# dsmyl6/OpenPyStruct

Hardware: AMD Instinct MI355X
Metric: beam FE solves/s (100-elem, batched) (higher is better)
Workload: dtype f64

## Files before the change

### openpystruct_amd/csrc/beam_fat.hip

```cpp
#include <hip/hip_runtime.h>
#include <stdint.h>

#include <type_traits>

#include "../../include/openpystruct_amd.h"
#include "beam_io.hpp"

namespace opsamd {

template <int PM>
struct FatAcc {
  const double* tab;
  const double* sI;
  const double* sF;
  FixPair bits;
  __device__ __forceinline__ ElemIn elem(int i) const {
    return ElemIn{tab[i], tab[PM + i], tab[2 * PM + i], tab[3 * PM + i], tab[4 * PM + i], tab[5 * PM + i], sI[i], sF[i]};
  }
  __device__ __forceinline__ FixPair fixbits() const { return bits; }
  __device__ __forceinline__ void fence() const { __asm__ volatile("" ::: "memory"); }
};

template <int M, bool FAT>
struct RowOut {
  double* sV; double* sM; double* sv;
  double th[M];
  double vr[FAT ? 1 : M];
  __device__ __forceinline__ void elem(int i, double Vv, double Mv) { sV[i] = Vv; sM[i] = Mv; }
  __device__ __forceinline__ void node(int i, double vv, double tt) {
    if constexpr (FAT) sv[i] = vv; else vr[i] = vv;
    th[i] = tt;
  }
};
template <int M, bool FAT>
struct ParkH {
  double* hx; double* hy;
  Vec2 r[FAT ? 1 : M];
  __device__ __forceinline__ void put(int i, const Vec2& h) {
    if constexpr (FAT) { hx[i] = h.x; hy[i] = h.y; } else r[i] = h;
  }
  __device__ __forceinline__ Vec2 get(int i) const {
    if constexpr (FAT) return Vec2{hx[i], hy[i]}; else return r[i];
  }
};

#ifdef OPS_AMD_TRACE
#define FAT_STAMP(k) (__builtin_amdgcn_sched_barrier(0), stamps[k] = __builtin_amdgcn_s_memrealtime(), __builtin_amdgcn_sched_barrier(0))
#else
#define FAT_STAMP(k) ((void)0)
#endif

struct FatIface {
  const IfacePiece* grp;
  __device__ __forceinline__ IfacePiece piece(int k) const { return grp[k]; }
  __device__ __forceinline__ Mat2 cup(int k) const { return grp[k].cup; }
  __device__ __forceinline__ void fence() const { __asm__ volatile("" ::: "memory"); }
};

template <int P, int M, bool RZ, bool FAT, int PF>
__device__ __forceinline__ void row_solve_lanes(const FatAcc<P * M>& acc, int g, int j, int& bad, RowOut<M, FAT>& out, ParkH<M, FAT>& hs,
                                                IfacePiece* pieces, unsigned lane, unsigned long long* stamps) {
  SegState<M> st;
  std::conditional_t<P == 16 && M == 7, KeepD<M>, KeepNone> keep;
  __asm__ volatile("" ::: "memory");
  seg_condense_pf<M, RZ>(st, acc, bad, keep);
  __asm__ volatile("" ::: "memory");
  FAT_STAMP(6);
  Vec2 uL, uR{0.0, 0.0};
  if constexpr (FAT) {
    pieces[lane] = make_piece<M, RZ>(st, acc.bits);
    __asm__ volatile("" ::: "memory");
    Vec2 u[P];
    iface_thomas<P>(FatIface{pieces + g * P}, u, bad);
    uL = u[0];
#pragma unroll
    for (int k = 1; k < P; ++k) {
      if (j == k) uL = u[k];
      if (j + 1 == k) uR = u[k];
    }
  } else {
    using X = Xch<P>;
    IfaceRow row;
    {
      const Mat2 cup = masked_cup<M, RZ>(st, acc.bits);
      const Sym2 pc = X::template from_minus<1>(st.Scc, (int)lane, j);
      const Vec2 pg = X::template from_minus<1>(st.gc, (int)lane, j);
      const Mat2 pb = X::template from_minus<1>(cup, (int)lane, j);
      row = make_row<M, RZ>(st, cup, pc, pg, pb, acc.bits);
    }
    cr_forward<P, 1>(row, (int)lane, j, bad);
    const Sym2 G = inv_spd(row.D, bad);
    uL = mul(G, row.f);
    if (j != 0) uL = Vec2{0.0, 0.0};
    cr_backward<P, cr_top_level(P)>(row, G, uL, (int)lane, j);
    uR = X::template from_plus<1>(uL, (int)lane, j);
  }
  __asm__ volatile("" ::: "memory");
  FAT_STAMP(7);
  seg_solve_pf<M, RZ, PF>(st, acc, uL, uR, out, hs, keep);
}

struct WordPick {
  bool q1, q2, q3;
  unsigned r;
  __device__ __forceinline__ explicit WordPick(int e0) : q1((e0 >> 5) == 1), q2((e0 >> 5) == 2), q3((e0 >> 5) == 3), r((unsigned)e0 & 31u) {}
};
__device__ __forceinline__ unsigned mask_window(unsigned long long lo, unsigned long long hi, const WordPick& w) {
  const unsigned w0 = (unsigned)lo, w1 = (unsigned)(lo >> 32), w2 = (unsigned)hi, w3 = (unsigned)(hi >> 32);
  unsigned a = w0, b = w1;
  a = w.q1 ? w1 : a;  b = w.q1 ? w2 : b;
  a = w.q2 ? w2 : a;  b = w.q2 ? w3 : b;
  a = w.q3 ? w3 : a;  b = w.q3 ? 0u : b;
  return __builtin_amdgcn_alignbit(b, a, w.r);
}

template <int P, int M, int WPS, bool FAT, bool SIZING>
__device__ __forceinline__ void beam_rows_body(const RowsHead& p, const RowsTail& t, const SizingArgs* sz) {
  constexpr int BPW = 64 / P;
  constexpr int LIVE = BPW * P;
  constexpr int PM = P * M;
  constexpr int NT = (PM + 63) / 64;
  constexpr int ROWS = BPW * PM;
  static_assert(PM <= 128 && PM % 2 == 0 && M + 1 <= 32, "row tiling limits");
  static_assert(FAT || (16 % P == 0 && LIVE == 64), "the lean mapping exchanges over DPP rows");
  constexpr int PF = FAT ? 3 : 1;
#ifdef OPS_AMD_ST
  constexpr int ST = OPS_AMD_ST;
#else
  constexpr int ST = 16;
#endif
  __shared__ double s_tab[6 * PM];
  __shared__ __attribute__((aligned(16))) double s_a[ROWS];
  __shared__ __attribute__((aligned(16))) double s_b[ROWS];
  __shared__ __attribute__((aligned(16))) double s_m[FAT ? ROWS : 2];
  __shared__ __attribute__((aligned(16))) double s_v[FAT ? ROWS : 2];
  __shared__ double s_dummy[M];
  static_assert((6 * PM + (FAT ? 4 : 2) * ROWS + M + 4) * 8 <= 160 * 1024 / (4 * WPS), "LDS per one-wave workgroup");
  static_assert(!FAT || (WPS == 1 && (6 * PM + 4 * ROWS) * 8 > 32 * 1024), "the fat tiling relies on LDS to keep a fifth wave off the CU");

  const unsigned lane = threadIdx.x;
  unsigned long long stamps[8] = {0, 0, 0, 0, 0, 0, 0, 0};
  FAT_STAMP(0);
  const int Ne = p.Ne, N = p.Ne + 1;
  const long I_bs = p.I_bs, Fy_bs = p.Fy_bs;
  const long beam0 = (long)blockIdx.x * BPW;
  const int nb = (p.B - beam0 < BPW) ? (int)(p.B - beam0) : BPW;
  if (SIZING && t.active) {
    unsigned any = 0;
    for (int b = 0; b < nb; ++b) any |= t.active[beam0 + b];
    if (!any) return;
  }
  const double tE = p.E[0], tw = p.wy[0];
  __builtin_amdgcn_sched_barrier(0);
  double tx0[NT], tx1[NT];
  {
    const __amdgpu_buffer_rsrc_t rx = make_rsrc(p.x, (unsigned)N * 8u);
#pragma unroll
    for (int k = 0; k < NT; ++k) {
      const unsigned e = lane + 64u * k;
      tx0[k] = buf_load_d(rx, e * 8u);
      tx1[k] = buf_load_d(rx, e * 8u + 8u);
    }
  }
  const int g_raw = lane / P, j = lane - g_raw * P, e0 = j * M;
  const bool live = (int)lane < LIVE;
  const int g = live ? g_raw : BPW - 1;
  const int hE = Ne >> 1, hN = N >> 1;
  double2 rI[BPW], rF[BPW];
  double tI = 0.0, tF = 0.0;
  {
    const __amdgpu_buffer_rsrc_t rsF = make_rsrc(p.Fy + beam0 * Fy_bs, (unsigned)(((long)(nb - 1) * Fy_bs + N) * 8));
    const unsigned oobF = (int)lane < hN ? lane * 16u : 0x40000000u;
    const unsigned tb = lane < (unsigned)nb ? lane : 0u;
    if constexpr (SIZING) {
      const __amdgpu_buffer_rsrc_t rsI = make_rsrc(static_cast<const float*>(p.I) + beam0 * Ne, (unsigned)(nb * Ne) * 4u);
      const unsigned oobI = (int)lane < hE ? lane * 8u : 0x40000000u;
#pragma unroll
      for (int b = 0; b < BPW; ++b) {
        const float2 f = __builtin_bit_cast(float2, __builtin_amdgcn_raw_buffer_load_b64(rsI, (int)((unsigned)(b * Ne) * 4u + oobI), 0, 0));
        rI[b] = make_double2((double)f.x, (double)f.y);
        rF[b] = buf_load_d2(rsF, (unsigned)(b * Fy_bs * 8) + oobF);
      }
      if (Ne & 1) tI = (double)__builtin_bit_cast(float, __builtin_amdgcn_raw_buffer_load_b32(rsI, (int)((tb * Ne + Ne - 1) * 4u), 0, 0));
    } else {
      const __amdgpu_buffer_rsrc_t rsI = make_rsrc(static_cast<const double*>(p.I) + beam0 * I_bs, (unsigned)(((long)(nb - 1) * I_bs + Ne) * 8));
      const unsigned oobI = (int)lane < hE ? lane * 16u : 0x40000000u;
#pragma unroll
      for (int b = 0; b < BPW; ++b) {
        rI[b] = buf_load_d2(rsI, (unsigned)(b * I_bs * 8) + oobI);
        rF[b] = buf_load_d2(rsF, (unsigned)(b * Fy_bs * 8) + oobF);
      }
      if (Ne & 1) tI = buf_load_d(rsI, (unsigned)((tb * I_bs + Ne - 1) * 8));
    }
    if (N & 1) tF = buf_load_d(rsF, (unsigned)((tb * Fy_bs + N - 1) * 8));
  }
  FAT_STAMP(5);
  unsigned char fb0, fb1;
  {
    const __amdgpu_buffer_rsrc_t rf = make_rsrc(t.fix, (unsigned)N);
    fb0 = __builtin_amdgcn_raw_buffer_load_b8(rf, (int)lane, 0, 0);
    fb1 = __builtin_amdgcn_raw_buffer_load_b8(rf, (int)(lane + 64u), 0, 0);
  }
#pragma unroll
  for (int k = 0; k < NT; ++k) {
    const unsigned e = lane + 64u * k;
    if (64 * (k + 1) <= Ne) {
      const double L = tx1[k] - tx0[k];
      const double rl = fast_rcp(L);
      const double c2 = 2.0 * tE * rl, pw = 0.5 * tw * L;
      const double c6 = 3.0 * c2 * rl, c12 = 2.0 * c6 * rl;
      const double mw = pw * L * (1.0 / 6.0);
      s_tab[0 * PM + e] = c2;  s_tab[1 * PM + e] = c6;  s_tab[2 * PM + e] = c12;
      s_tab[3 * PM + e] = rl;  s_tab[4 * PM + e] = pw;  s_tab[5 * PM + e] = mw;
    } else if (e < (unsigned)PM) {
      const bool real = (int)e < Ne, pad = (int)e > Ne;
      const double L = tx1[k] - tx0[k];
      const double rl0 = fast_rcp(real ? L : 1.0);
      const double c2r = 2.0 * tE * rl0, pwr = 0.5 * tw * L;
      const double rl = real ? rl0 : (pad ? 1.0 : 0.0);
      const double c2 = real ? c2r : (pad ? 2.0 : 0.0);
      const double c6 = 3.0 * c2 * rl, c12 = 2.0 * c6 * rl;
      const double pw = real ? pwr : 0.0, mw = pw * L * (1.0 / 6.0);
      s_tab[0 * PM + e] = c2;  s_tab[1 * PM + e] = c6;  s_tab[2 * PM + e] = c12;
      s_tab[3 * PM + e] = rl;  s_tab[4 * PM + e] = pw;  s_tab[5 * PM + e] = mw;
    }
  }
  FixPair bits;
  bool any_rz;
  {
    const unsigned long long v0 = __ballot(fb0 & 1), v1 = __ballot(fb1 & 1);
    const unsigned long long r0 = __ballot(fb0 & 2), r1 = __ballot(fb1 & 2);
    any_rz = (r0 | r1) != 0ull;
    const WordPick pick(e0);
    bits.v = mask_window(v0, v1, pick) & ((2u << M) - 1u);
    bits.t = any_rz ? mask_window(r0, r1, pick) & ((2u << M) - 1u) : 0u;
  }

  if (lane < M) s_dummy[lane] = 0.0;
#pragma unroll
  for (int k = 0; k < (ROWS / 2 + 63) / 64; ++k) {
    const unsigned idx = lane + 64u * k;
    if (k + 1 < (ROWS / 2 + 63) / 64 || idx < ROWS / 2) *reinterpret_cast<double2*>(&s_a[2 * idx]) = make_double2(1.0, 1.0);
  }
#pragma unroll
  for (int b = 0; b < BPW; ++b) {
    if ((int)lane < (b < nb ? hE : 0)) *reinterpret_cast<double2*>(&s_a[b * PM + 2 * lane]) = rI[b];
    if (lane < PM / 2) *reinterpret_cast<double2*>(&s_b[b * PM + 2 * lane]) = rF[b];
  }
  if ((Ne & 1) && (int)lane < nb) s_a[lane * PM + Ne - 1] = tI;
  if ((N & 1) && (int)lane < nb) s_b[lane * PM + N - 1] = tF;
  __syncthreads();
  FAT_STAMP(1);

  FatAcc<PM> acc;
  acc.tab = &s_tab[e0];
  acc.sI = &s_a[g * PM + e0];
  acc.sF = &s_b[g * PM + e0];
  acc.bits = bits;
  int bad = 0;
  RowOut<M, FAT> out;
  out.sV = live ? &s_b[g * PM + e0] : s_dummy;
  out.sM = live ? (FAT ? &s_m[g * PM + e0] : &s_a[g * PM + e0]) : s_dummy;
  out.sv = (FAT && live) ? &s_v[g * PM + e0] : s_dummy;
  ParkH<M, FAT> hs;
  hs.hx = out.sM; hs.hy = out.sv;
  static_assert(!FAT || 64 * sizeof(IfacePiece) <= ROWS * 8, "the interface pieces borrow the moment rows");
  IfacePiece* const pieces = reinterpret_cast<IfacePiece*>(s_m);
  if (any_rz) row_solve_lanes<P, M, true, FAT, PF>(acc, g, j, bad, out, hs, pieces, lane, stamps);
  else        row_solve_lanes<P, M, false, FAT, PF>(acc, g, j, bad, out, hs, pieces, lane, stamps);
  FAT_STAMP(2);

  const unsigned long long bal = __ballot(bad != 0 && live);
  const unsigned long long grp = (P == 64 ? ~0ull : ((1ull << (P % 64)) - 1ull)) << (g * P);
  const bool gbad = (bal & grp) != 0ull;
  if (bal != 0ull && gbad && live) {
    const double qnan = __builtin_nan("");
#pragma unroll
    for (int i = 0; i < M; ++i) {
      out.sV[i] = qnan; out.sM[i] = qnan; out.th[i] = qnan;
      if constexpr (FAT) out.sv[i] = qnan; else out.vr[i] = qnan;
    }
  }
  if (j == 0 && live && g < nb && t.status)
    __hip_atomic_store(&t.status[beam0 + g], gbad ? 1 : 0, __ATOMIC_RELAXED, __HIP_MEMORY_SCOPE_AGENT);
  double* const sth = live ? &s_a[g * PM + e0] : s_dummy;
  if constexpr (FAT) {
#pragma unroll
    for (int i = 0; i < M; ++i) sth[i] = out.th[i];
  }
  wave_lds_fence();
  if constexpr (SIZING) {
    static_assert(!SIZING || !FAT, "the fused epoch uses the lean mapping");
    CaseRegs<2> cr[BPW];
    bool on[BPW];
#pragma unroll
    for (int gb = 0; gb < BPW; ++gb) {
      on[gb] = gb < nb && sz->active[beam0 + gb] != 0;
      if (on[gb]) load_case<2>((int)lane, beam0 + gb, Ne, *sz, cr[gb]);
    }
#pragma unroll
    for (int gb = 0; gb < BPW; ++gb) {
      if (!on[gb]) continue;
      const double* Vb = &s_b[gb * PM];
      const double* Mb = &s_a[gb * PM];
      step_case<2>((int)lane, beam0 + gb, Ne, *sz, cr[gb], [&](int e) { return (float)Vb[e]; }, [&](int e) { return (float)Mb[e]; });
    }
    return;
  }

  const bool two = t.v != nullptr;
  auto read_rows = [&](double2 (&r)[BPW], double& tail, const double* s, int n_) {
    const unsigned lrow = (int)lane < (n_ >> 1) ? lane : 0u;
#pragma unroll
    for (int b = 0; b < BPW; ++b) r[b] = *reinterpret_cast<const double2*>(&s[b * PM + 2 * lrow]);
    tail = s[((int)lane < nb ? lane : 0u) * PM + n_ - 1];
  };
  auto store_rows = [&](auto aux, double* dst, const double2 (&r)[BPW], double tail, int n_) {
    constexpr int AUX = decltype(aux)::value;
    const __amdgpu_buffer_rsrc_t rs = make_rsrc(dst + beam0 * n_, (unsigned)(nb * n_) * 8u);
    const unsigned off = (int)lane < (n_ >> 1) ? lane * 16u : 0x40000000u;
#pragma unroll
    for (int b = 0; b < BPW; ++b)
      buf_store_d2<AUX>(rs, (unsigned)(b * n_) * 8u + off, r[b]);
    if ((n_ & 1) && (int)lane < nb) buf_store_d<AUX>(rs, (unsigned)(lane * n_ + n_ - 1) * 8u, tail);
  };
  auto all_rows = [&](auto aux) {
    double2 ra[BPW], rb[BPW];
    double ta, tb;
    read_rows(ra, ta, s_b, Ne);
    read_rows(rb, tb, FAT ? s_m : s_a, Ne);
    if constexpr (FAT) {
      store_rows(aux, t.V, ra, ta, Ne);
      if (two) read_rows(ra, ta, s_v, N);
      store_rows(aux, t.M, rb, tb, Ne);
      if (two) {
        read_rows(rb, tb, s_a, N);
        store_rows(aux, t.v, ra, ta, N);
        store_rows(aux, t.theta, rb, tb, N);
      }
    } else {
      if (two) {
        wave_lds_fence();
        double* const svv = live ? &s_b[g * PM + e0] : s_dummy;
#pragma unroll
        for (int i = 0; i < M; ++i) { svv[i] = out.vr[i]; sth[i] = out.th[i]; }
      }
      store_rows(aux, t.V, ra, ta, Ne);
      store_rows(aux, t.M, rb, tb, Ne);
      if (two) {
        wave_lds_fence();
        read_rows(ra, ta, s_b, N);
        read_rows(rb, tb, s_a, N);
        store_rows(aux, t.v, ra, ta, N);
        store_rows(aux, t.theta, rb, tb, N);
      }
    }
  };
  if (t.stream_out) all_rows(std::integral_constant<int, 2>{});
  else              all_rows(std::integral_constant<int, ST>{});
#ifdef OPS_AMD_TRACE
  if (t.trace && lane == 0) {
    FAT_STAMP(3);
    stamps[4] = __builtin_amdgcn_s_getreg((4 << 0) | (0 << 6) | ((16 - 1) << 11));
    unsigned long long* q = t.trace + 8 * (unsigned long long)blockIdx.x;
#pragma unroll
    for (int k = 0; k < 8; ++k) q[k] = stamps[k];
  }
#endif
}

template <int P, int M, int WPS, bool FAT>
__global__ __launch_bounds__(64, WPS) void beam_rows_kernel(int Ne, int B, const void* I, const double* Fy, unsigned I_bs, unsigned Fy_bs,
                                                           const double* x, const double* E, const double* wy, const RowsTail t) {
  beam_rows_body<P, M, WPS, FAT, false>(RowsHead{Ne, B, I, Fy, I_bs, Fy_bs, x, E, wy}, t, nullptr);
}
template <int P, int M, int WPS>
__global__ __launch_bounds__(64, WPS) void beam_rows_sizing_kernel(const RowsHead h, const RowsTail t, const SizingArgs sz) {
  beam_rows_body<P, M, WPS, false, true>(h, t, &sz);
}

const FatTiling kFatTilings[] = {
    {6, 17, "beam_rows_kernel<6, 17, 1, true>"},
    {16, 7, "beam_rows_kernel<16, 7, 3, false>"},
    {8, 13, "beam_rows_kernel<8, 13, 2, false>"},
};
const int kNumFatTilings = sizeof(kFatTilings) / sizeof(kFatTilings[0]);

static RowsHead rows_head(const BeamParams& p, const void* I) { return RowsHead{p.Ne, p.B, I, p.Fy, (unsigned)p.I_bs, (unsigned)p.Fy_bs, p.x, p.E, p.wy}; }
static RowsTail rows_tail(const BeamParams& p) { return RowsTail{p.fix, p.v, p.theta, p.V, p.M, p.status, p.active, p.stream_out, p.trace}; }
static void launch_rows(void (*kernel)(int, int, const void*, const double*, unsigned, unsigned, const double*, const double*, const double*, RowsTail),
                        unsigned grid, hipStream_t stream, const BeamParams& p) {
  const RowsHead h = rows_head(p, p.I);
  hipLaunchKernelGGL(kernel, dim3(grid), dim3(64), 0, stream, h.Ne, h.B, h.I, h.Fy, h.I_bs, h.Fy_bs, h.x, h.E, h.wy, rows_tail(p));
}

hipError_t launch_fat_sizing(const BeamParams& p, const SizingArgs& sz, int P, int M, hipStream_t stream) {
  const unsigned grid = (unsigned)((p.B + 64 / P - 1) / (64 / P));
  if (P == 16 && M == 7) hipLaunchKernelGGL((beam_rows_sizing_kernel<16, 7, 3>), dim3(grid), dim3(64), 0, stream, rows_head(p, p.I32), rows_tail(p), sz);
  else return hipErrorInvalidValue;
  return hipGetLastError();
}

hipError_t launch_fat(const BeamParams& p, int P, int M, hipStream_t stream) {
  const int bpw = 64 / P;
  const unsigned grid = (unsigned)((p.B + bpw - 1) / bpw);
  if (P == 6 && M == 17) launch_rows(beam_rows_kernel<6, 17, 1, true>, grid, stream, p);
  else if (P == 16 && M == 7) launch_rows(beam_rows_kernel<16, 7, 3, false>, grid, stream, p);
  else if (P == 8 && M == 13) launch_rows(beam_rows_kernel<8, 13, 2, false>, grid, stream, p);
  else return hipErrorInvalidValue;
  return hipGetLastError();
}

}
```

### openpystruct_amd/csrc/beam_io.hpp

```cpp
#pragma once
#include <hip/hip_runtime.h>
#include <stdint.h>

#include "beam_math.hpp"
#include "lane_common.hpp"
#include "sizing_math.hpp"

namespace opsamd {

struct BeamParams {
  int B, Ne;
  const double* x;  long x_bs;
  const double* E;  long E_bs;
  const double* I;  long I_bs;
  const uint8_t* fix; long fix_bs;
  const double* Fy; long Fy_bs;
  const double* wy; long wy_bs;
  double* v; double* theta; double* V; double* M;
  int32_t* status;
  const float* I32;
  const uint8_t* active;
  int stream_out;
  int f32_forces;
  int dense;
  unsigned long long* trace;
  unsigned magic_ne, magic_n;
};

struct RowsHead {
  int Ne, B;
  const void* I;
  const double* Fy;
  unsigned I_bs, Fy_bs;
  const double* x; const double* E; const double* wy;
};
struct RowsTail {
  const uint8_t* fix;
  double* v; double* theta; double* V; double* M;
  int32_t* status;
  const uint8_t* active;
  int stream_out;
  unsigned long long* trace;
};

struct FatTiling { int P, M; const char* name; };
extern const FatTiling kFatTilings[];
extern const int kNumFatTilings;
hipError_t launch_fat(const BeamParams& p, int P, int M, hipStream_t stream);
hipError_t launch_fat_sizing(const BeamParams& p, const SizingArgs& sz, int P, int M, hipStream_t stream);

template <int SRC>
__device__ __forceinline__ double row_bcast(double x) {
  return __builtin_amdgcn_update_dpp(0.0, x, 0x150 + SRC, 0xF, 0xF, true);
}

template <int P>
struct Xch {
  template <int S>
  static __device__ __forceinline__ double from_minus(double x, int lane, int j) {
    if constexpr (P <= 16 && S < 16) {
      const double r = dpp_mov<0x110 + S>(x);
      if constexpr (P < 16) return j >= S ? r : 0.0;
      return r;
    } else {
      const double r = __shfl(x, lane - S, 64);
      return j >= S ? r : 0.0;
    }
  }
  template <int S>
  static __device__ __forceinline__ double from_plus(double x, int lane, int j) {
    if constexpr (P <= 16 && S < 16) {
      const double r = dpp_mov<0x100 + S>(x);
      if constexpr (P < 16) return j + S < P ? r : 0.0;
      return r;
    } else {
      const double r = __shfl(x, lane + S, 64);
      return j + S < P ? r : 0.0;
    }
  }
  template <int S>
  static __device__ __forceinline__ double top_plus(double x, int lane, int j) {
    if constexpr (P == 16) return row_bcast<S>(x); else return from_plus<S>(x, lane, j);
  }
  template <int S>
  static __device__ __forceinline__ double top_minus(double x, int lane, int j) {
    if constexpr (P == 16) return row_bcast<0>(x); else return from_minus<S>(x, lane, j);
  }
  template <int S> static __device__ __forceinline__ Sym2 from_minus(const Sym2& s, int l, int j) {
    return Sym2{from_minus<S>(s.a, l, j), from_minus<S>(s.b, l, j), from_minus<S>(s.c, l, j)};
  }
  template <int S> static __device__ __forceinline__ Mat2 from_minus(const Mat2& m, int l, int j) {
    return Mat2{from_minus<S>(m.a, l, j), from_minus<S>(m.b, l, j), from_minus<S>(m.c, l, j), from_minus<S>(m.d, l, j)};
  }
  template <int S> static __device__ __forceinline__ Vec2 from_minus(const Vec2& u, int l, int j) {
    return Vec2{from_minus<S>(u.x, l, j), from_minus<S>(u.y, l, j)};
  }
  template <int S> static __device__ __forceinline__ Sym2 from_plus(const Sym2& s, int l, int j) {
    return Sym2{from_plus<S>(s.a, l, j), from_plus<S>(s.b, l, j), from_plus<S>(s.c, l, j)};
  }
  template <int S> static __device__ __forceinline__ Mat2 from_plus(const Mat2& m, int l, int j) {
    return Mat2{from_plus<S>(m.a, l, j), from_plus<S>(m.b, l, j), from_plus<S>(m.c, l, j), from_plus<S>(m.d, l, j)};
  }
  template <int S> static __device__ __forceinline__ Vec2 from_plus(const Vec2& u, int l, int j) {
    return Vec2{from_plus<S>(u.x, l, j), from_plus<S>(u.y, l, j)};
  }
  template <int S> static __device__ __forceinline__ Sym2 top_plus(const Sym2& s, int l, int j) {
    return Sym2{top_plus<S>(s.a, l, j), top_plus<S>(s.b, l, j), top_plus<S>(s.c, l, j)};
  }
  template <int S> static __device__ __forceinline__ Vec2 top_plus(const Vec2& u, int l, int j) {
    return Vec2{top_plus<S>(u.x, l, j), top_plus<S>(u.y, l, j)};
  }
  template <int S> static __device__ __forceinline__ Vec2 top_minus(const Vec2& u, int l, int j) {
    return Vec2{top_minus<S>(u.x, l, j), top_minus<S>(u.y, l, j)};
  }
};

template <int P>
struct XchPerm {
  static __device__ __forceinline__ double fetch(double x, int src_lane) {
    const unsigned long long u = __builtin_bit_cast(unsigned long long, x);
    const int lo = __builtin_amdgcn_ds_bpermute(src_lane << 2, (int)(unsigned)u);
    const int hi = __builtin_amdgcn_ds_bpermute(src_lane << 2, (int)(unsigned)(u >> 32));
    return __builtin_bit_cast(double, ((unsigned long long)(unsigned)hi << 32) | (unsigned)lo);
  }
  template <int S> static __device__ __forceinline__ double from_minus(double x, int lane, int j) { return fetch(x, j >= S ? lane - S : lane); }
  template <int S> static __device__ __forceinline__ double from_plus(double x, int lane, int j) { return fetch(x, j + S < P ? lane + S : lane); }
  template <int S> static __device__ __forceinline__ Sym2 from_minus(const Sym2& s, int l, int j) {
    return Sym2{from_minus<S>(s.a, l, j), from_minus<S>(s.b, l, j), from_minus<S>(s.c, l, j)};
  }
  template <int S> static __device__ __forceinline__ Mat2 from_minus(const Mat2& m, int l, int j) {
    return Mat2{from_minus<S>(m.a, l, j), from_minus<S>(m.b, l, j), from_minus<S>(m.c, l, j), from_minus<S>(m.d, l, j)};
  }
  template <int S> static __device__ __forceinline__ Vec2 from_minus(const Vec2& u, int l, int j) {
    return Vec2{from_minus<S>(u.x, l, j), from_minus<S>(u.y, l, j)};
  }
  template <int S> static __device__ __forceinline__ Sym2 from_plus(const Sym2& s, int l, int j) {
    return Sym2{from_plus<S>(s.a, l, j), from_plus<S>(s.b, l, j), from_plus<S>(s.c, l, j)};
  }
  template <int S> static __device__ __forceinline__ Mat2 from_plus(const Mat2& m, int l, int j) {
    return Mat2{from_plus<S>(m.a, l, j), from_plus<S>(m.b, l, j), from_plus<S>(m.c, l, j), from_plus<S>(m.d, l, j)};
  }
  template <int S> static __device__ __forceinline__ Vec2 from_plus(const Vec2& u, int l, int j) {
    return Vec2{from_plus<S>(u.x, l, j), from_plus<S>(u.y, l, j)};
  }
  template <int S> static __device__ __forceinline__ Sym2 top_plus(const Sym2& s, int l, int j) { return from_plus<S>(s, l, j); }
  template <int S> static __device__ __forceinline__ Vec2 top_plus(const Vec2& u, int l, int j) { return from_plus<S>(u, l, j); }
  template <int S> static __device__ __forceinline__ Vec2 top_minus(const Vec2& u, int l, int j) { return from_minus<S>(u, l, j); }
};

template <int P, int S, class X = Xch<P>, bool EARLY = false>
__device__ __forceinline__ void cr_forward(IfaceRow& row, int lane, int j, int& bad) {
  if constexpr (S < P) {
    constexpr bool LAST = (2 * S >= P);
    const bool act = cr_active(j, S);
    if constexpr (LAST) {
      const Sym2 G = inv_spd(row.D, bad);
      const Sym2 Gp = X::template top_plus<S>(G, lane, j);
      const Vec2 fp = X::template top_plus<S>(row.f, lane, j);
      Mat2 Cup = S > 1 ? neg(row.Cup) : row.Cup;
      if (act) cr_absorb<true>(row.D, row.f, Cup, Gp, Mat2{0, 0, 0, 0}, fp);
    } else if constexpr (EARLY) {
      const Vec2 fm = X::template from_minus<S>(row.f, lane, j);
      const Vec2 fp = X::template from_plus<S>(row.f, lane, j);
      const Mat2 Am = X::template from_minus<S>(row.Alow, lane, j);
      const Mat2 Cp = X::template from_plus<S>(row.Cup, lane, j);
      const Sym2 G = inv_spd(row.D, bad);
      const Sym2 Gm = X::template from_minus<S>(G, lane, j);
      const Sym2 Gp = X::template from_plus<S>(G, lane, j);
      if (act) {
        cr_absorb_held<(S > 1)>(row.D, row.f, row.Alow, Gm, Am, fm);
        cr_absorb_held<(S > 1)>(row.D, row.f, row.Cup, Gp, Cp, fp);
      }
    } else {
      const Sym2 G = inv_spd(row.D, bad);
      const Sym2 Gm = X::template from_minus<S>(G, lane, j);
      const Vec2 fm = X::template from_minus<S>(row.f, lane, j);
      const Mat2 Am = X::template from_minus<S>(row.Alow, lane, j);
      const Vec2 fp = X::template from_plus<S>(row.f, lane, j);
      if (act) cr_absorb_held<(S > 1)>(row.D, row.f, row.Alow, Gm, Am, fm);
      const Sym2 Gp = X::template from_plus<S>(G, lane, j);
      const Mat2 Cp = X::template from_plus<S>(row.Cup, lane, j);
      if (act) cr_absorb_held<(S > 1)>(row.D, row.f, row.Cup, Gp, Cp, fp);
    }
    cr_forward<P, 2 * S, X, EARLY>(row, lane, j, bad);
  }
}
template <int P, int S, class X = Xch<P>>
__device__ __forceinline__ void cr_backward(const IfaceRow& held, const Sym2& G, Vec2& u, int lane, int j) {
  if constexpr (S >= 1) {
    const IfaceRow row{S > 1 ? neg(held.Alow) : held.Alow, S > 1 ? neg(held.Cup) : held.Cup, held.D, held.f};
    if constexpr (2 * S >= P) {
      const Vec2 um = X::template top_minus<S>(u, lane, j);
      if (cr_frozen(j, S)) u = cr_back_low(row, G, um);
    } else {
      const Vec2 um = X::template from_minus<S>(u, lane, j);
      const Vec2 up = X::template from_plus<S>(u, lane, j);
      if (cr_frozen(j, S)) u = cr_back(row, G, um, up);
    }
    cr_backward<P, S / 2, X>(held, G, u, lane, j);
  }
}
constexpr int cr_top_level(int P) { int s = 1; while (2 * s < P) s *= 2; return s; }

__device__ __forceinline__ void wave_lds_fence() {
  __builtin_amdgcn_s_waitcnt(0xC07F);
  __asm__ volatile("" ::: "memory");
  __builtin_amdgcn_wave_barrier();
}

typedef int v4i __attribute__((ext_vector_type(4)));
typedef int v2i __attribute__((ext_vector_type(2)));
__device__ __forceinline__ __amdgpu_buffer_rsrc_t make_rsrc(const void* base, unsigned bytes) {
  return __builtin_amdgcn_make_buffer_rsrc(const_cast<void*>(base), 0, (int)bytes, 0x00020000);
}
__device__ __forceinline__ double2 buf_load_d2(__amdgpu_buffer_rsrc_t r, unsigned byte_off) {
#ifndef OPS_AMD_LD_AUX
#define OPS_AMD_LD_AUX 0
#endif
  const v4i v = __builtin_amdgcn_raw_buffer_load_b128(r, (int)byte_off, 0, OPS_AMD_LD_AUX);
  return __builtin_bit_cast(double2, v);
}
__device__ __forceinline__ double buf_load_d(__amdgpu_buffer_rsrc_t r, unsigned byte_off) {
  const v2i v = __builtin_amdgcn_raw_buffer_load_b64(r, (int)byte_off, 0, 0);
  return __builtin_bit_cast(double, v);
}
template <int AUX>
__device__ __forceinline__ void buf_store_d2(__amdgpu_buffer_rsrc_t r, unsigned byte_off, double2 x) {
  __builtin_amdgcn_raw_buffer_store_b128(__builtin_bit_cast(v4i, x), r, (int)byte_off, 0, AUX);
}
template <int AUX>
__device__ __forceinline__ void buf_store_d(__amdgpu_buffer_rsrc_t r, unsigned byte_off, double x) {
  __builtin_amdgcn_raw_buffer_store_b64(__builtin_bit_cast(v2i, x), r, (int)byte_off, 0, AUX);
}

}
```

### openpystruct_amd/csrc/beam_math.hpp

```cpp
#pragma once

#if defined(__HIPCC__)
#define BEAM_HD __host__ __device__ __forceinline__
#else
#define BEAM_HD inline
#endif

namespace opsamd {

struct Sym2 { double a, b, c; };
struct Mat2 { double a, b, c, d; };
struct Vec2 { double x, y; };

BEAM_HD double fast_rcp(double d) {
#if defined(__HIP_DEVICE_COMPILE__)
  double r = __builtin_amdgcn_rcp(d);
  double e = __builtin_fma(-d, r, 1.0);
  r = __builtin_fma(r, e, r);
  e = __builtin_fma(-d, r, 1.0);
  r = __builtin_fma(r, e, r);
  return r;
#else
  return 1.0 / d;
#endif
}

BEAM_HD Sym2 inv_spd(const Sym2& s, int& bad) {
  const double bb = s.b * s.b;
  const double det = __builtin_fma(s.a, s.c, -bb) + __builtin_fma(-s.b, s.b, bb);
  bad |= !(s.a > 0.0) | !(det > 0.0);
  const double r = fast_rcp(det);
  return Sym2{s.c * r, -s.b * r, s.a * r};
}

BEAM_HD Mat2 mul(const Mat2& m, const Sym2& s) {
  return Mat2{__builtin_fma(m.a, s.a, m.b * s.b), __builtin_fma(m.a, s.b, m.b * s.c),
              __builtin_fma(m.c, s.a, m.d * s.b), __builtin_fma(m.c, s.b, m.d * s.c)};
}
BEAM_HD Mat2 mulT(const Mat2& m, const Sym2& s) {
  return Mat2{__builtin_fma(m.a, s.a, m.c * s.b), __builtin_fma(m.a, s.b, m.c * s.c),
              __builtin_fma(m.b, s.a, m.d * s.b), __builtin_fma(m.b, s.b, m.d * s.c)};
}
BEAM_HD Mat2 neg_mul(const Mat2& p, const Mat2& q) {
  return Mat2{-__builtin_fma(p.a, q.a, p.b * q.c), -__builtin_fma(p.a, q.b, p.b * q.d),
              -__builtin_fma(p.c, q.a, p.d * q.c), -__builtin_fma(p.c, q.b, p.d * q.d)};
}
BEAM_HD Sym2 sub_mulT(const Sym2& s, const Mat2& p, const Mat2& q) {
  return Sym2{__builtin_fma(-p.a, q.a, __builtin_fma(-p.b, q.b, s.a)),
              __builtin_fma(-p.a, q.c, __builtin_fma(-p.b, q.d, s.b)),
              __builtin_fma(-p.c, q.c, __builtin_fma(-p.d, q.d, s.c))};
}
BEAM_HD Sym2 sub_mul(const Sym2& s, const Mat2& p, const Mat2& q) {
  return Sym2{__builtin_fma(-p.a, q.a, __builtin_fma(-p.b, q.c, s.a)),
              __builtin_fma(-p.a, q.b, __builtin_fma(-p.b, q.d, s.b)),
              __builtin_fma(-p.c, q.b, __builtin_fma(-p.d, q.d, s.c))};
}
BEAM_HD Vec2 sub_mul(const Vec2& v, const Mat2& p, const Vec2& u) {
  return Vec2{__builtin_fma(-p.a, u.x, __builtin_fma(-p.b, u.y, v.x)),
              __builtin_fma(-p.c, u.x, __builtin_fma(-p.d, u.y, v.y))};
}
BEAM_HD Vec2 sub_mulT(const Vec2& v, const Mat2& p, const Vec2& u) {
  return Vec2{__builtin_fma(-p.a, u.x, __builtin_fma(-p.c, u.y, v.x)),
              __builtin_fma(-p.b, u.x, __builtin_fma(-p.d, u.y, v.y))};
}
BEAM_HD Vec2 mul(const Sym2& s, const Vec2& u) {
  return Vec2{__builtin_fma(s.a, u.x, s.b * u.y), __builtin_fma(s.b, u.x, s.c * u.y)};
}

struct ElemK { double kA, kB, kC, kD; };

BEAM_HD ElemK elem_k(double c2, double c6, double c12, double Ie) {
  const double kD = c2 * Ie;
  return ElemK{c12 * Ie, c6 * Ie, kD + kD, kD};
}

template <bool RZ>
struct Flags {
  double v, dv;
  double t, dt;
};
template <bool RZ>
BEAM_HD Flags<RZ> node_flags(unsigned long long bits, int node) {
  const bool fv = (bits >> (2 * node)) & 1ull, ft = RZ && ((bits >> (2 * node + 1)) & 1ull);
  return Flags<RZ>{fv ? 0.0 : 1.0, fv ? 1.0 : 0.0, ft ? 0.0 : 1.0, ft ? 1.0 : 0.0};
}
struct FixPair { unsigned v, t; };
template <bool RZ>
BEAM_HD Flags<RZ> node_flags(const FixPair& bits, int node) {
  const bool fv = (bits.v >> node) & 1u, ft = RZ && ((bits.t >> node) & 1u);
  return Flags<RZ>{fv ? 0.0 : 1.0, fv ? 1.0 : 0.0, ft ? 0.0 : 1.0, ft ? 1.0 : 0.0};
}
template <bool RZ>
BEAM_HD Sym2 mask_node(const Sym2& s, const Flags<RZ>& c) {
  if (RZ) return Sym2{__builtin_fma(c.v, s.a, c.dv), (c.v * c.t) * s.b, __builtin_fma(c.t, s.c, c.dt)};
  return Sym2{__builtin_fma(c.v, s.a, c.dv), c.v * s.b, s.c};
}
template <bool RZ>
BEAM_HD Vec2 mask_vec(const Vec2& g, const Flags<RZ>& c) {
  if (RZ) return Vec2{c.v * g.x, c.t * g.y};
  return Vec2{c.v * g.x, g.y};
}
template <bool RZ>
BEAM_HD Mat2 mask_cols(const Mat2& m, const Flags<RZ>& c) {
  if (RZ) return Mat2{m.a * c.v, m.b * c.t, m.c * c.v, m.d * c.t};
  return Mat2{m.a * c.v, m.b, m.c * c.v, m.d};
}
template <bool RZ>
BEAM_HD Mat2 mask_rows(const Mat2& m, const Flags<RZ>& c) {
  if (RZ) return Mat2{m.a * c.v, m.b * c.v, m.c * c.t, m.d * c.t};
  return Mat2{m.a * c.v, m.b * c.v, m.c, m.d};
}

template <bool RZ>
BEAM_HD Sym2 proj_inv(const Sym2& s, const Flags<RZ>& c, int& bad) {
  const Sym2 g = inv_spd(mask_node(s, c), bad);
  if (RZ) return Sym2{c.v * g.a, g.b, c.t * g.c};
  return Sym2{c.v * g.a, g.b, g.c};
}

#if defined(__HIP_DEVICE_COMPILE__)
#define BEAM_PIN_F64(x) __asm__ volatile("" : "+v"(x))
#define BEAM_PIN_I32(x) __asm__ volatile("" : "+v"(x))
#else
#define BEAM_PIN_F64(x) ((void)0)
#define BEAM_PIN_I32(x) ((void)0)
#endif

template <int M>
struct SegState {
  Sym2 Ginv[M];
  Sym2 SLL, Scc;
  Mat2 SLc;
  Vec2 gL, gc;
};

template <int M, bool RZ, class Acc>
BEAM_HD void seg_condense(SegState<M>& s, const Acc& acc, int& bad) {
  const unsigned long long fb = acc.fixbits();
  {
    const ElemK k = elem_k(acc.c2(0), acc.c6(0), acc.c12(0), acc.Ie(0));
    s.SLL = Sym2{k.kA, k.kB, k.kC};
    s.SLc = Mat2{-k.kA, k.kB, -k.kB, k.kD};
    s.Scc = Sym2{k.kA, -k.kB, k.kC};
    s.gL = Vec2{acc.pw(0) + acc.Fy(0), acc.mw(0)};
    s.gc = Vec2{acc.pw(0), -acc.mw(0)};
  }
#pragma unroll
  for (int i = 1; i < M; ++i) {
    acc.fence();
    const Flags<RZ> c = node_flags<RZ>(fb, i);
    const ElemK k = elem_k(acc.c2(i), acc.c6(i), acc.c12(i), acc.Ie(i));
    const double pw = acc.pw(i), mw = acc.mw(i);
    const Sym2 G = proj_inv(Sym2{s.Scc.a + k.kA, s.Scc.b + k.kB, s.Scc.c + k.kC}, c, bad);
    const Vec2 gi{s.gc.x + pw + acc.Fy(i), s.gc.y + mw};
    const Mat2 Kr{-k.kA, k.kB, -k.kB, k.kD};
    s.Ginv[i] = G;
    const Mat2 Pm = mul(s.SLc, G);
    const Mat2 Qm = mulT(Kr, G);
    s.SLL = sub_mulT(s.SLL, Pm, s.SLc);
    s.gL = sub_mul(s.gL, Pm, gi);
    s.SLc = neg_mul(Pm, Kr);
    s.Scc = sub_mul(Sym2{k.kA, -k.kB, k.kC}, Qm, Kr);
    s.gc = sub_mul(Vec2{pw, -mw}, Qm, gi);
  }
}

struct IfaceRow {
  Mat2 Alow, Cup;
  Sym2 D;
  Vec2 f;
};

template <int M, bool RZ, class Bits>
BEAM_HD Mat2 masked_cup(const SegState<M>& s, const Bits& fixbits) {
  return mask_cols(mask_rows(s.SLc, node_flags<RZ>(fixbits, 0)), node_flags<RZ>(fixbits, M));
}

template <int M, bool RZ, class Bits>
BEAM_HD IfaceRow make_row(const SegState<M>& s, const Mat2& ownCup, const Sym2& prevC, const Vec2& prevg,
                          const Mat2& prevCup, const Bits& fixbits) {
  const Flags<RZ> c = node_flags<RZ>(fixbits, 0);
  IfaceRow r;
  r.D = mask_node(Sym2{s.SLL.a + prevC.a, s.SLL.b + prevC.b, s.SLL.c + prevC.c}, c);
  r.f = mask_vec(Vec2{s.gL.x + prevg.x, s.gL.y + prevg.y}, c);
  r.Alow = Mat2{prevCup.a, prevCup.c, prevCup.b, prevCup.d};
  r.Cup = ownCup;
  return r;
}

BEAM_HD bool cr_active(int j, int s) { return (j & (2 * s - 1)) == 0; }
BEAM_HD bool cr_frozen(int j, int s) { return (j & (2 * s - 1)) == s; }

template <bool LAST>
BEAM_HD void cr_absorb(Sym2& D, Vec2& f, Mat2& Aside, const Sym2& G, const Mat2& Afar, const Vec2& fn) {
  const Mat2 al = mul(Aside, G);
  D = sub_mulT(D, al, Aside);
  f = sub_mul(f, al, fn);
  if (!LAST) Aside = neg_mul(al, Afar);
}
BEAM_HD Mat2 neg(const Mat2& m) { return Mat2{-m.a, -m.b, -m.c, -m.d}; }
template <bool NEG>
BEAM_HD void cr_absorb_held(Sym2& D, Vec2& f, Mat2& held, const Sym2& G, const Mat2& held_far, const Vec2& fn) {
  const Mat2 Aside = NEG ? neg(held) : held, Afar = NEG ? neg(held_far) : held_far;
  const Mat2 al = mul(Aside, G);
  D = sub_mulT(D, al, Aside);
  f = sub_mul(f, al, fn);
  held = Mat2{__builtin_fma(al.a, Afar.a, al.b * Afar.c), __builtin_fma(al.a, Afar.b, al.b * Afar.d),
              __builtin_fma(al.c, Afar.a, al.d * Afar.c), __builtin_fma(al.c, Afar.b, al.d * Afar.d)};
}
template <bool LAST>
BEAM_HD void cr_eliminate(IfaceRow& r, const Sym2& Gm, const Mat2& Am, const Vec2& fm, const Sym2& Gp,
                          const Mat2& Cp, const Vec2& fp) {
  cr_absorb<LAST>(r.D, r.f, r.Alow, Gm, Am, fm);
  cr_absorb<LAST>(r.D, r.f, r.Cup, Gp, Cp, fp);
}

BEAM_HD Vec2 cr_back(const IfaceRow& r, const Sym2& G, const Vec2& um, const Vec2& up) {
  return mul(G, sub_mul(sub_mul(r.f, r.Alow, um), r.Cup, up));
}

BEAM_HD Vec2 cr_back_low(const IfaceRow& r, const Sym2& G, const Vec2& um) {
  return mul(G, sub_mul(r.f, r.Alow, um));
}

template <int M, bool RZ, class Acc, class Out>
BEAM_HD void seg_solve(const SegState<M>& s, const Acc& acc, const Vec2& uL, const Vec2& uR, Out& out) {
  (void)acc.fixbits();
  Vec2 h[M];
  {
    const ElemK k0 = elem_k(acc.c2(0), acc.c6(0), acc.c12(0), acc.Ie(0));
    Vec2 carry = sub_mulT(Vec2{acc.pw(0), -acc.mw(0)}, Mat2{-k0.kA, k0.kB, -k0.kB, k0.kD}, uL);
#pragma unroll
    for (int i = 1; i < M; ++i) {
      acc.fence();
      const double pw = acc.pw(i), mw = acc.mw(i);
      h[i] = Vec2{carry.x + pw + acc.Fy(i), carry.y + mw};
      if (i + 1 < M) {
        const ElemK k = elem_k(acc.c2(i), acc.c6(i), acc.c12(i), acc.Ie(i));
        const Vec2 y = mul(s.Ginv[i], h[i]);
        carry = sub_mulT(Vec2{pw, -mw}, Mat2{-k.kA, k.kB, -k.kB, k.kD}, y);
      }
    }
  }
  Vec2 un = uR;
#pragma unroll
  for (int i = M - 1; i >= 0; --i) {
    acc.fence();
    const ElemK k = elem_k(acc.c2(i), acc.c6(i), acc.c12(i), acc.Ie(i));
    Vec2 ui;
    if (i > 0) {
      ui = mul(s.Ginv[i], sub_mul(h[i], Mat2{-k.kA, k.kB, -k.kB, k.kD}, un));
    } else {
      ui = uL;
    }
    {
      const double rl = acc.rL(i), mw = acc.mw(i);
      const double chord = (un.x - ui.x) * rl;
      const double p1 = ui.y - chord, p2 = un.y - chord;
      const double q1 = __builtin_fma(k.kC, p1, __builtin_fma(k.kD, p2, -mw));
      const double q2 = __builtin_fma(k.kD, p1, __builtin_fma(k.kC, p2, mw));
      out.elem(i, __builtin_fma(q1 + q2, rl, -acc.pw(i)), q1);
    }
    out.node(i, ui.x, ui.y);
    un = ui;
  }
}

struct ElemIn { double c2, c6, c12, rl, pw, mw, Ie, Fy; };

struct KeepNone {
  BEAM_HD void put(int, const ElemK&) {}
  BEAM_HD ElemK get(int, const ElemIn& e) const { return elem_k(e.c2, e.c6, e.c12, e.Ie); }
};
template <int M>
struct KeepD {
  double kD[M];
  BEAM_HD void put(int i, const ElemK& k) { kD[i] = k.kD; }
  BEAM_HD ElemK get(int i, const ElemIn& e) const { return ElemK{e.c12 * e.Ie, e.c6 * e.Ie, kD[i] + kD[i], kD[i]}; }
};

template <int M, bool RZ, class Acc, class Keep>
BEAM_HD void seg_condense_pf(SegState<M>& s, const Acc& acc, int& bad, Keep& keep) {
  const auto fb = acc.fixbits();
  ElemIn nx = acc.elem(0);
  {
    const ElemIn e = nx;
    if (M > 1) nx = acc.elem(1);
    acc.fence();
    const ElemK k = elem_k(e.c2, e.c6, e.c12, e.Ie);
    keep.put(0, k);
    s.SLL = Sym2{k.kA, k.kB, k.kC};
    s.SLc = Mat2{-k.kA, k.kB, -k.kB, k.kD};
    s.Scc = Sym2{k.kA, -k.kB, k.kC};
    s.gL = Vec2{e.pw + e.Fy, e.mw};
    s.gc = Vec2{e.pw, -e.mw};
  }
#pragma unroll
  for (int i = 1; i < M; ++i) {
    const ElemIn e = nx;
    if (i + 1 < M) nx = acc.elem(i + 1);
    acc.fence();
    const Flags<RZ> c = node_flags<RZ>(fb, i);
    const ElemK k = elem_k(e.c2, e.c6, e.c12, e.Ie);
    keep.put(i, k);
    const double pw = e.pw, mw = e.mw;
    const Sym2 G = proj_inv(Sym2{s.Scc.a + k.kA, s.Scc.b + k.kB, s.Scc.c + k.kC}, c, bad);
    const Vec2 gi{s.gc.x + pw + e.Fy, s.gc.y + mw};
    const Mat2 Kr{-k.kA, k.kB, -k.kB, k.kD};
    s.Ginv[i] = G;
    const Mat2 Pm = mul(s.SLc, G);
    const Mat2 Qm = mulT(Kr, G);
    s.SLL = sub_mulT(s.SLL, Pm, s.SLc);
    s.gL = sub_mul(s.gL, Pm, gi);
    s.SLc = neg_mul(Pm, Kr);
    s.Scc = sub_mul(Sym2{k.kA, -k.kB, k.kC}, Qm, Kr);
    s.gc = sub_mul(Vec2{pw, -mw}, Qm, gi);
    BEAM_PIN_F64(s.SLL.a); BEAM_PIN_F64(s.SLL.b); BEAM_PIN_F64(s.SLL.c); BEAM_PIN_F64(s.gL.x); BEAM_PIN_F64(s.gL.y);
    BEAM_PIN_I32(bad);
  }
}

template <int M, bool RZ, class Acc>
BEAM_HD void seg_condense_pf(SegState<M>& s, const Acc& acc, int& bad) {
  KeepNone keep;
  seg_condense_pf<M, RZ>(s, acc, bad, keep);
}

template <int M, bool RZ, int PF, class Acc, class Out, class Hs, class Keep>
BEAM_HD void seg_solve_pf(const SegState<M>& s, const Acc& acc, const Vec2& uL, const Vec2& uR, Out& out, Hs& hs, const Keep& keep) {
  static_assert(PF >= 1 && PF <= 4, "prefetch distance");
  {
    ElemIn q[PF];
#pragma unroll
    for (int d = 0; d < PF; ++d) q[d] = acc.elem(d < M ? d : M - 1);
    const ElemIn e0 = q[0];
    if (PF < M) q[0] = acc.elem(PF);
    acc.fence();
    const ElemK k0 = keep.get(0, e0);
    Vec2 carry = sub_mulT(Vec2{e0.pw, -e0.mw}, Mat2{-k0.kA, k0.kB, -k0.kB, k0.kD}, uL);
#pragma unroll
    for (int i = 1; i < M; ++i) {
      const ElemIn e = q[i % PF];
      if (i + PF < M) q[i % PF] = acc.elem(i + PF);
      acc.fence();
      const double pw = e.pw, mw = e.mw;
      const Vec2 hi{carry.x + pw + e.Fy, carry.y + mw};
      hs.put(i, hi);
      if (i + 1 < M) {
        const ElemK k = keep.get(i, e);
        const Vec2 y = mul(s.Ginv[i], hi);
        carry = sub_mulT(Vec2{pw, -mw}, Mat2{-k.kA, k.kB, -k.kB, k.kD}, y);
      }
    }
  }
  Vec2 un = uR;
  ElemIn q[PF];
  Vec2 hq[PF];
#pragma unroll
  for (int d = 0; d < PF; ++d) {
    const int i = M - 1 - d;
    q[(M - 1 - d + PF) % PF] = acc.elem(i >= 0 ? i : 0);
    hq[(M - 1 - d + PF) % PF] = hs.get(i >= 1 ? i : (M > 1 ? 1 : 0));
  }
#pragma unroll
  for (int i = M - 1; i >= 0; --i) {
    const ElemIn e = q[i % PF];
    const Vec2 hi = hq[i % PF];
    if (i - PF >= 0) q[i % PF] = acc.elem(i - PF);
    if (i - PF >= 1) hq[i % PF] = hs.get(i - PF);
    acc.fence();
    const ElemK k = keep.get(i, e);
    Vec2 ui;
    if (i > 0) {
      ui = mul(s.Ginv[i], sub_mul(hi, Mat2{-k.kA, k.kB, -k.kB, k.kD}, un));
    } else {
      ui = uL;
    }
    {
      const double rl = e.rl, mw = e.mw;
      const double chord = (un.x - ui.x) * rl;
      const double p1 = ui.y - chord, p2 = un.y - chord;
      const double q1 = __builtin_fma(k.kC, p1, __builtin_fma(k.kD, p2, -mw));
      const double q2 = __builtin_fma(k.kD, p1, __builtin_fma(k.kC, p2, mw));
      out.elem(i, __builtin_fma(q1 + q2, rl, -e.pw), q1);
    }
    out.node(i, ui.x, ui.y);
    un = ui;
  }
}
template <int M, bool RZ, int PF, class Acc, class Out, class Hs>
BEAM_HD void seg_solve_pf(const SegState<M>& s, const Acc& acc, const Vec2& uL, const Vec2& uR, Out& out, Hs& hs) {
  seg_solve_pf<M, RZ, PF>(s, acc, uL, uR, out, hs, KeepNone{});
}

struct alignas(16) IfacePiece {
  Sym2 Dl; Vec2 fl;
  Sym2 Dr; Vec2 fr;
  Mat2 cup;
};
template <int M, bool RZ, class Bits>
BEAM_HD IfacePiece make_piece(const SegState<M>& s, const Bits& fixbits) {
  const Flags<RZ> c0 = node_flags<RZ>(fixbits, 0), cM = node_flags<RZ>(fixbits, M);
  IfacePiece p;
  p.Dl = mask_node(s.SLL, c0);
  p.fl = mask_vec(s.gL, c0);
  p.Dr = RZ ? Sym2{cM.v * s.Scc.a, (cM.v * cM.t) * s.Scc.b, cM.t * s.Scc.c} : Sym2{cM.v * s.Scc.a, cM.v * s.Scc.b, s.Scc.c};
  p.fr = mask_vec(s.gc, cM);
  p.cup = mask_cols(mask_rows(s.SLc, c0), cM);
  return p;
}
template <int P, class Rd, class Bad>
BEAM_HD void iface_thomas(const Rd& rd, Vec2 (&u)[P], Bad& bad) {
  Sym2 G[P];
  Vec2 fp[P];
  IfacePiece nx = rd.piece(0);
  Sym2 Dr{0.0, 0.0, 0.0};
  Vec2 fr{0.0, 0.0};
  Mat2 cp{0.0, 0.0, 0.0, 0.0};
#pragma unroll
  for (int k = 0; k < P; ++k) {
    const IfacePiece e = nx;
    if (k + 1 < P) nx = rd.piece(k + 1);
    rd.fence();
    Sym2 D{e.Dl.a + Dr.a, e.Dl.b + Dr.b, e.Dl.c + Dr.c};
    Vec2 f{e.fl.x + fr.x, e.fl.y + fr.y};
    if (k > 0) {
      const Mat2 A{cp.a, cp.c, cp.b, cp.d};
      const Mat2 W = mul(A, G[k - 1]);
      D = sub_mulT(D, W, A);
      f = sub_mul(f, W, fp[k - 1]);
    }
    G[k] = inv_spd(D, bad);
    fp[k] = f;
    Dr = e.Dr; fr = e.fr; cp = e.cup;
  }
  u[P - 1] = mul(G[P - 1], fp[P - 1]);
  Mat2 cn = P > 1 ? rd.cup(P - 2) : Mat2{0.0, 0.0, 0.0, 0.0};
#pragma unroll
  for (int k = P - 2; k >= 0; --k) {
    const Mat2 c = cn;
    if (k > 0) cn = rd.cup(k - 1);
    rd.fence();
    u[k] = mul(G[k], sub_mul(fp[k], c, u[k + 1]));
  }
}

}
```

Measured before the change: 963.2 million.

## Track singular pivots as wave-uniform ballot mask and use row broadcasts in CR

Replaces the per-lane int error flag with a scalar 64-bit ballot mask accumulated at each SPD inverse. This avoids holding a VGPR flag and removes the final ballot. Adds below_minus/below_plus exchange helpers, which for P=16 use DPP row broadcasts instead of generic lane shuffles in some cyclic-reduction steps. The cost is extra ballot instructions at every inverse, and the broadcast path is only correct when the lane pattern matches. The trace build also records an extra hardware register.

```diff
diff --git a/openpystruct_amd/csrc/beam_fat.hip b/openpystruct_amd/csrc/beam_fat.hip
--- a/openpystruct_amd/csrc/beam_fat.hip
+++ b/openpystruct_amd/csrc/beam_fat.hip
@@ -58,7 +58,7 @@
 };
 
 template <int P, int M, bool RZ, bool FAT, int PF>
-__device__ __forceinline__ void row_solve_lanes(const FatAcc<P * M>& acc, int g, int j, int& bad, RowOut<M, FAT>& out, ParkH<M, FAT>& hs,
+__device__ __forceinline__ void row_solve_lanes(const FatAcc<P * M>& acc, int g, int j, BadMask& bad, RowOut<M, FAT>& out, ParkH<M, FAT>& hs,
                                                 IfacePiece* pieces, unsigned lane, unsigned long long* stamps) {
   SegState<M> st;
   std::conditional_t<P == 16 && M == 7, KeepD<M>, KeepNone> keep;
@@ -257,7 +257,7 @@
   acc.sI = &s_a[g * PM + e0];
   acc.sF = &s_b[g * PM + e0];
   acc.bits = bits;
-  int bad = 0;
+  BadMask bad{0ull};
   RowOut<M, FAT> out;
   out.sV = live ? &s_b[g * PM + e0] : s_dummy;
   out.sM = live ? (FAT ? &s_m[g * PM + e0] : &s_a[g * PM + e0]) : s_dummy;
@@ -270,7 +270,7 @@
   else        row_solve_lanes<P, M, false, FAT, PF>(acc, g, j, bad, out, hs, pieces, lane, stamps);
   FAT_STAMP(2);
 
-  const unsigned long long bal = __ballot(bad != 0 && live);
+  const unsigned long long bal = bad.m & (LIVE == 64 ? ~0ull : (1ull << (LIVE % 64)) - 1ull);
   const unsigned long long grp = (P == 64 ? ~0ull : ((1ull << (P % 64)) - 1ull)) << (g * P);
   const bool gbad = (bal & grp) != 0ull;
   if (bal != 0ull && gbad && live) {
@@ -361,7 +361,8 @@
 #ifdef OPS_AMD_TRACE
   if (t.trace && lane == 0) {
     FAT_STAMP(3);
-    stamps[4] = __builtin_amdgcn_s_getreg((4 << 0) | (0 << 6) | ((16 - 1) << 11));
+    stamps[4] = __builtin_amdgcn_s_getreg((4 << 0) | (0 << 6) | ((16 - 1) << 11)) |
+                ((unsigned long long)__builtin_amdgcn_s_getreg((20 << 0) | (0 << 6) | ((4 - 1) << 11)) << 16);
     unsigned long long* q = t.trace + 8 * (unsigned long long)blockIdx.x;
 #pragma unroll
     for (int k = 0; k < 8; ++k) q[k] = stamps[k];
diff --git a/openpystruct_amd/csrc/beam_io.hpp b/openpystruct_amd/csrc/beam_io.hpp
--- a/openpystruct_amd/csrc/beam_io.hpp
+++ b/openpystruct_amd/csrc/beam_io.hpp
@@ -49,6 +49,12 @@
 hipError_t launch_fat(const BeamParams& p, int P, int M, hipStream_t stream);
 hipError_t launch_fat_sizing(const BeamParams& p, const SizingArgs& sz, int P, int M, hipStream_t stream);
 
+struct BadMask { unsigned long long m; };
+__device__ __forceinline__ void note_bad(BadMask& bad, bool first, bool second) {
+  bad.m |= __builtin_amdgcn_ballot_w64(first) | __builtin_amdgcn_ballot_w64(second);
+}
+__device__ __forceinline__ void pin_bad(BadMask& bad) { __asm__ volatile("" : "+s"(bad.m)); }
+
 template <int SRC>
 __device__ __forceinline__ double row_bcast(double x) {
   return __builtin_amdgcn_update_dpp(0.0, x, 0x150 + SRC, 0xF, 0xF, true);
@@ -86,6 +92,14 @@
   static __device__ __forceinline__ double top_minus(double x, int lane, int j) {
     if constexpr (P == 16) return row_bcast<0>(x); else return from_minus<S>(x, lane, j);
   }
+  template <int S>
+  static __device__ __forceinline__ double below_minus(double x, int lane, int j) {
+    if constexpr (P == 16 && 4 * S == P) return row_bcast<S>(x); else return from_minus<S>(x, lane, j);
+  }
+  template <int S>
+  static __device__ __forceinline__ double below_plus(double x, int lane, int j) {
+    if constexpr (P == 16 && 4 * S == P) return row_bcast<2 * S>(x); else return from_plus<S>(x, lane, j);
+  }
   template <int S> static __device__ __forceinline__ Sym2 from_minus(const Sym2& s, int l, int j) {
     return Sym2{from_minus<S>(s.a, l, j), from_minus<S>(s.b, l, j), from_minus<S>(s.c, l, j)};
   }
@@ -112,6 +126,18 @@
   }
   template <int S> static __device__ __forceinline__ Vec2 top_minus(const Vec2& u, int l, int j) {
     return Vec2{top_minus<S>(u.x, l, j), top_minus<S>(u.y, l, j)};
+  }
+  template <int S> static __device__ __forceinline__ Sym2 below_minus(const Sym2& s, int l, int j) {
+    return Sym2{below_minus<S>(s.a, l, j), below_minus<S>(s.b, l, j), below_minus<S>(s.c, l, j)};
+  }
+  template <int S> static __device__ __forceinline__ Mat2 below_minus(const Mat2& m, int l, int j) {
+    return Mat2{below_minus<S>(m.a, l, j), below_minus<S>(m.b, l, j), below_minus<S>(m.c, l, j), below_minus<S>(m.d, l, j)};
+  }
+  template <int S> static __device__ __forceinline__ Vec2 below_minus(const Vec2& u, int l, int j) {
+    return Vec2{below_minus<S>(u.x, l, j), below_minus<S>(u.y, l, j)};
+  }
+  template <int S> static __device__ __forceinline__ Vec2 below_plus(const Vec2& u, int l, int j) {
+    return Vec2{below_plus<S>(u.x, l, j), below_plus<S>(u.y, l, j)};
   }
 };
 
@@ -146,10 +172,12 @@
   template <int S> static __device__ __forceinline__ Sym2 top_plus(const Sym2& s, int l, int j) { return from_plus<S>(s, l, j); }
   template <int S> static __device__ __forceinline__ Vec2 top_plus(const Vec2& u, int l, int j) { return from_plus<S>(u, l, j); }
   template <int S> static __device__ __forceinline__ Vec2 top_minus(const Vec2& u, int l, int j) { return from_minus<S>(u, l, j); }
-};
-
-template <int P, int S, class X = Xch<P>, bool EARLY = false>
-__device__ __forceinline__ void cr_forward(IfaceRow& row, int lane, int j, int& bad) {
+  template <int S, class T> static __device__ __forceinline__ T below_minus(const T& x, int l, int j) { return from_minus<S>(x, l, j); }
+  template <int S, class T> static __device__ __forceinline__ T below_plus(const T& x, int l, int j) { return from_plus<S>(x, l, j); }
+};
+
+template <int P, int S, class X = Xch<P>, bool EARLY = false, class Bad = int>
+__device__ __forceinline__ void cr_forward(IfaceRow& row, int lane, int j, Bad& bad) {
   if constexpr (S < P) {
     constexpr bool LAST = (2 * S >= P);
     const bool act = cr_active(j, S);
@@ -173,16 +201,16 @@
       }
     } else {
       const Sym2 G = inv_spd(row.D, bad);
-      const Sym2 Gm = X::template from_minus<S>(G, lane, j);
-      const Vec2 fm = X::template from_minus<S>(row.f, lane, j);
-      const Mat2 Am = X::template from_minus<S>(row.Alow, lane, j);
+      const Sym2 Gm = X::template below_minus<S>(G, lane, j);
+      const Vec2 fm = X::template below_minus<S>(row.f, lane, j);
+      const Mat2 Am = X::template below_minus<S>(row.Alow, lane, j);
       const Vec2 fp = X::template from_plus<S>(row.f, lane, j);
       if (act) cr_absorb_held<(S > 1)>(row.D, row.f, row.Alow, Gm, Am, fm);
       const Sym2 Gp = X::template from_plus<S>(G, lane, j);
       const Mat2 Cp = X::template from_plus<S>(row.Cup, lane, j);
       if (act) cr_absorb_held<(S > 1)>(row.D, row.f, row.Cup, Gp, Cp, fp);
     }
-    cr_forward<P, 2 * S, X, EARLY>(row, lane, j, bad);
+    cr_forward<P, 2 * S, X, EARLY, Bad>(row, lane, j, bad);
   }
 }
 template <int P, int S, class X = Xch<P>>
@@ -194,7 +222,7 @@
       if (cr_frozen(j, S)) u = cr_back_low(row, G, um);
     } else {
       const Vec2 um = X::template from_minus<S>(u, lane, j);
-      const Vec2 up = X::template from_plus<S>(u, lane, j);
+      const Vec2 up = X::template below_plus<S>(u, lane, j);
       if (cr_frozen(j, S)) u = cr_back(row, G, um, up);
     }
     cr_backward<P, S / 2, X>(held, G, u, lane, j);
diff --git a/openpystruct_amd/csrc/beam_math.hpp b/openpystruct_amd/csrc/beam_math.hpp
--- a/openpystruct_amd/csrc/beam_math.hpp
+++ b/openpystruct_amd/csrc/beam_math.hpp
@@ -25,10 +25,13 @@
 #endif
 }
 
-BEAM_HD Sym2 inv_spd(const Sym2& s, int& bad) {
+BEAM_HD void note_bad(int& bad, bool first, bool second) { bad |= first | second; }
+
+template <class Bad>
+BEAM_HD Sym2 inv_spd(const Sym2& s, Bad& bad) {
   const double bb = s.b * s.b;
   const double det = __builtin_fma(s.a, s.c, -bb) + __builtin_fma(-s.b, s.b, bb);
-  bad |= !(s.a > 0.0) | !(det > 0.0);
+  note_bad(bad, !(s.a > 0.0), !(det > 0.0));
   const double r = fast_rcp(det);
   return Sym2{s.c * r, -s.b * r, s.a * r};
 }
@@ -111,8 +114,8 @@
   return Mat2{m.a * c.v, m.b * c.v, m.c, m.d};
 }
 
-template <bool RZ>
-BEAM_HD Sym2 proj_inv(const Sym2& s, const Flags<RZ>& c, int& bad) {
+template <bool RZ, class Bad>
+BEAM_HD Sym2 proj_inv(const Sym2& s, const Flags<RZ>& c, Bad& bad) {
   const Sym2 g = inv_spd(mask_node(s, c), bad);
   if (RZ) return Sym2{c.v * g.a, g.b, c.t * g.c};
   return Sym2{c.v * g.a, g.b, g.c};
@@ -125,6 +128,7 @@
 #define BEAM_PIN_F64(x) ((void)0)
 #define BEAM_PIN_I32(x) ((void)0)
 #endif
+BEAM_HD void pin_bad(int& bad) { BEAM_PIN_I32(bad); (void)bad; }
 
 template <int M>
 struct SegState {
@@ -279,8 +283,8 @@
   BEAM_HD ElemK get(int i, const ElemIn& e) const { return ElemK{e.c12 * e.Ie, e.c6 * e.Ie, kD[i] + kD[i], kD[i]}; }
 };
 
-template <int M, bool RZ, class Acc, class Keep>
-BEAM_HD void seg_condense_pf(SegState<M>& s, const Acc& acc, int& bad, Keep& keep) {
+template <int M, bool RZ, class Acc, class Bad, class Keep>
+BEAM_HD void seg_condense_pf(SegState<M>& s, const Acc& acc, Bad& bad, Keep& keep) {
   const auto fb = acc.fixbits();
   ElemIn nx = acc.elem(0);
   {
@@ -316,12 +320,12 @@
     s.Scc = sub_mul(Sym2{k.kA, -k.kB, k.kC}, Qm, Kr);
     s.gc = sub_mul(Vec2{pw, -mw}, Qm, gi);
     BEAM_PIN_F64(s.SLL.a); BEAM_PIN_F64(s.SLL.b); BEAM_PIN_F64(s.SLL.c); BEAM_PIN_F64(s.gL.x); BEAM_PIN_F64(s.gL.y);
-    BEAM_PIN_I32(bad);
-  }
-}
-
-template <int M, bool RZ, class Acc>
-BEAM_HD void seg_condense_pf(SegState<M>& s, const Acc& acc, int& bad) {
+    pin_bad(bad);
+  }
+}
+
+template <int M, bool RZ, class Acc, class Bad>
+BEAM_HD void seg_condense_pf(SegState<M>& s, const Acc& acc, Bad& bad) {
   KeepNone keep;
   seg_condense_pf<M, RZ>(s, acc, bad, keep);
 }
```

Result: no change. 971.8 million (median of 4 runs) (+0.9%).
